# ZeayW/Multimodal-fusion-based-Pre-routing-Timing-Prediction-

Measured on AMD Instinct MI355X. Metric: train-step samples/sec, higher is better.
Workload: dtype bf16; 1 GPU; config B: 8 designs/step/GPU, 65536-node netlist, 64 levels, 256x256 tile, 1350 endpoints/design, UNet(max), bf16 operands / fp32 accumulate on the MFMA-bound contractions; U-Net activations and their gradients stored bf16, netlist tensors, statistics, parameters and gradients fp32; nodes=65536, levels=64, tile=256, endpoints_per_design=1350, cone_pruning=False, parallelism=dp1 (designs sharded, one all-reduce of the flat gradient per step), launch=one HIP graph replay per step (Adam inside)

## Files before the change

multimodal-fusion-based-pre-routing-timing-prediction-_amd/csrc/mlp_feat.hip:

```cpp
#include <stdlib.h>
#include "mlp_tile_bf16.h"
#include "tr_read.h"

namespace mmft {

int launch_slab_reduce(const float* slabs, int splits, long long elems, float* out, int accumulate, hipStream_t st);

__device__ __forceinline__ unsigned short mf_bf16(float v) { return (unsigned short)(pack_bf16(v, 0.f) & 0xffff); }

__device__ __forceinline__ bf16x8 mf_pack8(const float* v) {
  u32x4 p = {pack_bf16(v[0], v[1]), pack_bf16(v[2], v[3]), pack_bf16(v[4], v[5]), pack_bf16(v[6], v[7])};
  return __builtin_bit_cast(bf16x8, p);
}

__device__ __forceinline__ bf16x8 mf_w1_frag(const float* __restrict__ w1, int fin, int col, int k0) {
  float v[8];
#pragma unroll
  for (int t = 0; t < 8; ++t) v[t] = k0 + t < fin ? w1[(long long)col * fin + k0 + t] : 0.f;
  return mf_pack8(v);
}

struct FeatFwdArgs {
  const float* x;
  long long ldx;
  int row0, n, fin;
  const float *w1, *b1, *w2, *b2;
  float* out;
  long long ldout;
  int relu_out;
};

template <int KS>
__global__ void __launch_bounds__(512) mlp2_feat_fwd_kernel(FeatFwdArgs a) {
  constexpr int BM = 64, RT = BM / 16, XS = KS * 32 + 8, HS = L2_HD + 8;
  __shared__ __attribute__((aligned(16))) unsigned short xs[BM * XS];
  __shared__ __attribute__((aligned(16))) unsigned short hs[BM * HS];
  const int tid = threadIdx.x, lane = tid & 63, wave = tid >> 6;
  const int r16 = lane & 15, q = lane >> 4;
  bf16x8 w1f[2][KS], w2f[8];
#pragma unroll
  for (int j = 0; j < 2; ++j)
#pragma unroll
    for (int ks = 0; ks < KS; ++ks) w1f[j][ks] = mf_w1_frag(a.w1, a.fin, wave * 32 + j * 16 + r16, ks * 32 + q * 8);
#pragma unroll
  for (int ks = 0; ks < 8; ++ks) w2f[ks] = mf_pack8(a.w2 + (long long)(wave * 16 + r16) * L2_HD + ks * 32 + q * 8);
  const int nn2 = wave * 16 + q * 4;
  const f32x4 b2v = *reinterpret_cast<const f32x4*>(a.b2 + nn2);
  f32x4 b1v[2];
#pragma unroll
  for (int j = 0; j < 2; ++j) b1v[j] = *reinterpret_cast<const f32x4*>(a.b1 + wave * 32 + j * 16 + q * 4);
  constexpr int NXE = BM * KS * 32 / 512;
  float xr[NXE];
  auto request = [&](int tile) {
#pragma unroll
    for (int k = 0; k < NXE; ++k) {
      const int e = tid + k * 512, r = e / (KS * 32), kk = e % (KS * 32);
      const int m = tile * BM + r;
      xr[k] = (m < a.n && kk < a.fin) ? a.x[(long long)(a.row0 + m) * a.ldx + kk] : 0.f;
    }
  };
  const int ntiles = (a.n + BM - 1) / BM;
  if ((int)blockIdx.x < ntiles) request(blockIdx.x);
  for (int tile = blockIdx.x; tile < ntiles; tile += gridDim.x) {
    const int m0 = tile * BM;
#pragma unroll
    for (int k = 0; k < NXE; ++k) {
      const int e = tid + k * 512;
      xs[(e / (KS * 32)) * XS + e % (KS * 32)] = mf_bf16(xr[k]);
    }
    __syncthreads();
    if (tile + (int)gridDim.x < ntiles) request(tile + gridDim.x);
    f32x4 acc1[RT][2];
    tile_layer1<KS, RT>(acc1, w1f, xs, XS, r16, q);
#pragma unroll
    for (int i = 0; i < RT; ++i)
#pragma unroll
      for (int j = 0; j < 2; ++j) st_bf16x4(hs + (i * 16 + r16) * HS + wave * 32 + j * 16 + q * 4, relu4(acc1[i][j] + b1v[j]));
    __syncthreads();
    f32x4 acc2[RT];
#pragma unroll
    for (int i = 0; i < RT; ++i) acc2[i] = tile_layer2(w2f, hs, HS, r16, q, i);
#pragma unroll
    for (int i = 0; i < RT; ++i) {
      const int m = m0 + i * 16 + r16;
      if (m >= a.n) continue;
      f32x4 v = acc2[i] + b2v;
      if (a.relu_out) v = relu4(v);
      *reinterpret_cast<f32x4*>(a.out + (long long)(a.row0 + m) * a.ldout + nn2) = v;
    }
    __syncthreads();
  }
}

struct FeatBwdArgs {
  const float* g;
  long long ldg;
  const float* x;
  long long ldx;
  int row0, n, fin;
  const float *w1, *b1, *w2;
  float* slabs;
  long long slab;
};

template <int KS>
__global__ void __launch_bounds__(512) mlp2_feat_bwd_kernel(FeatBwdArgs a) {
  constexpr int BM = 32, KP = KS * 32, XS = KP + 16, GS = L2_D2 + 16, HS = L2_HD + 16, KB = KP / 16;
  extern __shared__ __attribute__((aligned(16))) unsigned short lds[];
  unsigned short* xs = lds;
  unsigned short* gs = xs + BM * XS;
  unsigned short* hs = gs + BM * GS;
  unsigned short* ds = hs + BM * HS;
  f32x4(*gred)[32] = reinterpret_cast<f32x4(*)[32]>(hs);
  const int tid = threadIdx.x, lane = tid & 63, wave = tid >> 6;
  const int r16 = lane & 15, q = lane >> 4;
  const int trr = tr_lane_row(lane), trc = tr_lane_col(lane);
  const f32x4 zero = {0.f, 0.f, 0.f, 0.f};

  bf16x8 w1f[2][KS], w2tf[2][4];
  f32x4 b1v[2];
#pragma unroll
  for (int j = 0; j < 2; ++j) {
    const int col = wave * 32 + j * 16 + r16;
#pragma unroll
    for (int ks = 0; ks < KS; ++ks) w1f[j][ks] = mf_w1_frag(a.w1, a.fin, col, ks * 32 + q * 8);
#pragma unroll
    for (int ks = 0; ks < 4; ++ks) {
      float v[8];
#pragma unroll
      for (int t = 0; t < 8; ++t) v[t] = a.w2[(long long)(ks * 32 + q * 8 + t) * L2_HD + col];
      w2tf[j][ks] = mf_pack8(v);
    }
    b1v[j] = *reinterpret_cast<const f32x4*>(a.b1 + wave * 32 + j * 16 + q * 4);
  }
  f32x4 dw2[2][8], dw1[2][KB], dsum[2], gsum = zero;
#pragma unroll
  for (int j = 0; j < 2; ++j) {
    dsum[j] = zero;
#pragma unroll
    for (int d = 0; d < 8; ++d) dw2[j][d] = zero;
#pragma unroll
    for (int k = 0; k < KB; ++k) dw1[j][k] = zero;
  }

  const int ntiles = (a.n + BM - 1) / BM;
  constexpr int NXE = BM * KP / 512;
  f32x4 gr[2];
  float xr[NXE];
  auto request = [&](int tile) {
    const int m0 = tile * BM;
#pragma unroll
    for (int it = 0; it < 2; ++it) {
      const int e = tid + it * 512, r = e >> 5, c = (e & 31) * 4;
      gr[it] = m0 + r < a.n ? *reinterpret_cast<const f32x4*>(a.g + (long long)(a.row0 + m0 + r) * a.ldg + c) : zero;
    }
#pragma unroll
    for (int k = 0; k < NXE; ++k) {
      const int e = tid + k * 512, r = e / KP, kk = e % KP;
      xr[k] = (m0 + r < a.n && kk < a.fin) ? a.x[(long long)(a.row0 + m0 + r) * a.ldx + kk] : 0.f;
    }
  };
  if ((int)blockIdx.x < ntiles) request(blockIdx.x);
  for (int tile = blockIdx.x; tile < ntiles; tile += gridDim.x) {
#pragma unroll
    for (int it = 0; it < 2; ++it) {
      const int e = tid + it * 512, r = e >> 5, c = (e & 31) * 4;
      const f32x4 v = gr[it];
      gsum += v;
      const unsigned lo = pack_bf16(v.x, v.y), hi = pack_bf16(v.z, v.w);
      *reinterpret_cast<unsigned long long*>(gs + r * GS + c) = ((unsigned long long)hi << 32) | lo;
    }
#pragma unroll
    for (int k = 0; k < NXE; ++k) {
      const int e = tid + k * 512, r = e / KP, kk = e % KP;
      xs[r * XS + kk] = mf_bf16(xr[k]);
    }
    __syncthreads();
    if (tile + (int)gridDim.x < ntiles) request(tile + gridDim.x);
    __syncthreads();
#pragma unroll
    for (int i = 0; i < 2; ++i) {
      f32x4 acc1[2] = {zero, zero}, acc3[2] = {zero, zero};
#pragma unroll
      for (int ks = 0; ks < KS; ++ks) {
        const bf16x8 xf = *reinterpret_cast<const bf16x8*>(xs + (i * 16 + r16) * XS + ks * 32 + q * 8);
#pragma unroll
        for (int j = 0; j < 2; ++j) acc1[j] = __builtin_amdgcn_mfma_f32_16x16x32_bf16(w1f[j][ks], xf, acc1[j], 0, 0, 0);
      }
#pragma unroll
      for (int ks = 0; ks < 4; ++ks) {
        const bf16x8 gf = *reinterpret_cast<const bf16x8*>(gs + (i * 16 + r16) * GS + ks * 32 + q * 8);
#pragma unroll
        for (int j = 0; j < 2; ++j) acc3[j] = __builtin_amdgcn_mfma_f32_16x16x32_bf16(w2tf[j][ks], gf, acc3[j], 0, 0, 0);
      }
      const int m = i * 16 + r16;
#pragma unroll
      for (int j = 0; j < 2; ++j) {
        const int nn = wave * 32 + j * 16 + q * 4;
        f32x4 hv = acc1[j] + b1v[j], dh = acc3[j];
#pragma unroll
        for (int t = 0; t < 4; ++t) {
          hv[t] = hv[t] > 0.f ? hv[t] : 0.f;
          dh[t] = hv[t] > 0.f ? dh[t] : 0.f;
        }
        dsum[j] += dh;
        const unsigned hl = pack_bf16(hv.x, hv.y), hh = pack_bf16(hv.z, hv.w);
        const unsigned dl = pack_bf16(dh.x, dh.y), dhh = pack_bf16(dh.z, dh.w);
        *reinterpret_cast<unsigned long long*>(hs + m * HS + nn) = ((unsigned long long)hh << 32) | hl;
        *reinterpret_cast<unsigned long long*>(ds + m * HS + nn) = ((unsigned long long)dhh << 32) | dl;
      }
    }
    __syncthreads();
#pragma unroll
    for (int j = 0; j < 2; ++j) {
      const int col0 = wave * 32 + j * 16;
      const bf16x8 hf = __builtin_bit_cast(bf16x8, tr_read_pair(hs + trr * HS + col0 + trc, 16 * HS));
      const bf16x8 df = __builtin_bit_cast(bf16x8, tr_read_pair(ds + trr * HS + col0 + trc, 16 * HS));
#pragma unroll
      for (int d = 0; d < 8; ++d) {
        const bf16x8 gf = __builtin_bit_cast(bf16x8, tr_read_pair(gs + trr * GS + d * 16 + trc, 16 * GS));
        dw2[j][d] = __builtin_amdgcn_mfma_f32_16x16x32_bf16(hf, gf, dw2[j][d], 0, 0, 0);
      }
#pragma unroll
      for (int k = 0; k < KB; ++k) {
        const bf16x8 xf = __builtin_bit_cast(bf16x8, tr_read_pair(xs + trr * XS + k * 16 + trc, 16 * XS));
        dw1[j][k] = __builtin_amdgcn_mfma_f32_16x16x32_bf16(df, xf, dw1[j][k], 0, 0, 0);
      }
    }
    __syncthreads();
  }

  float* sl = a.slabs + (long long)blockIdx.x * a.slab;
  float* s_dw1 = sl;
  float* s_db1 = s_dw1 + (long long)L2_HD * a.fin;
  float* s_dw2 = s_db1 + L2_HD;
  float* s_db2 = s_dw2 + (long long)L2_D2 * L2_HD;
#pragma unroll
  for (int j = 0; j < 2; ++j) {
    const int colq = wave * 32 + j * 16 + q * 4;
#pragma unroll
    for (int d = 0; d < 8; ++d) *reinterpret_cast<f32x4*>(s_dw2 + (long long)(d * 16 + r16) * L2_HD + colq) = dw2[j][d];
#pragma unroll
    for (int k = 0; k < KB; ++k) {
      const int kk = k * 16 + r16;
      if (kk < a.fin) {
#pragma unroll
        for (int t = 0; t < 4; ++t) s_dw1[(long long)(colq + t) * a.fin + kk] = dw1[j][k][t];
      }
    }
    f32x4 v = dsum[j];
#pragma unroll
    for (int o = 1; o < 16; o <<= 1) {
#pragma unroll
      for (int t = 0; t < 4; ++t) v[t] += __shfl_xor(v[t], o, 64);
    }
    if (r16 == 0) *reinterpret_cast<f32x4*>(s_db1 + colq) = v;
  }
  __syncthreads();
  gred[tid >> 5][tid & 31] = gsum;
  __syncthreads();
  if (tid < 32) {
    f32x4 v = gred[0][tid];
    for (int p = 1; p < 16; ++p) v += gred[p][tid];
    *reinterpret_cast<f32x4*>(s_db2 + tid * 4) = v;
  }
}

template <int KS>
constexpr int feat_bwd_lds() {
  constexpr int BM = 32, KP = KS * 32, XS = KP + 16, GS = L2_D2 + 16, HS = L2_HD + 16;
  return (BM * XS + BM * GS + 2 * BM * HS) * 2;
}

static inline long long feat_slab(int fin) { return (long long)L2_HD * fin + L2_HD + (long long)L2_D2 * L2_HD + L2_D2; }
static inline int feat_bwd_grid(int n) {
  int tiles = cdiv(n, 32);
  static int cap = getenv("MMFT_FEAT_BWD_GRID") ? atoi(getenv("MMFT_FEAT_BWD_GRID")) : 192;
  if (cap < 1) cap = 1;
  return tiles < cap ? (tiles < 1 ? 1 : tiles) : cap;
}

}

using namespace mmft;

extern "C" int mmft_mlp2_feat_fwd_bf16(const float* x, long long ldx, int row0, int n, int fin, const float* w1, const float* b1,
                                       const float* w2, const float* b2, float* out, long long ldout, int relu_out, int device,
                                       void* stream) {
  MMFT_REQUIRE(x && w1 && b1 && w2 && b2 && out, "mlp2_feat_fwd_bf16: null pointer");
  MMFT_REQUIRE(n >= 0 && row0 >= 0 && fin >= 1 && fin <= 64 && ldx >= fin, "mlp2_feat_fwd_bf16: bad sizes (fin <= 64)");
  MMFT_REQUIRE(ldout % 4 == 0 && aligned16(out) && aligned16(w2) && aligned16(b1) && aligned16(b2),
               "mlp2_feat_fwd_bf16: out / w2 / biases must be 16-byte aligned");
  if (n == 0) return MMFT_OK;
  DeviceGuard dg(device);
  FeatFwdArgs a{x, ldx, row0, n, fin, w1, b1, w2, b2, out, ldout, relu_out};
  const double fl = 2.0 * n * ((double)fin * L2_HD + (double)L2_HD * L2_D2), by = 4.0 * n * ((double)fin + L2_D2);
  int grid = cdiv(n, 64);
  if (grid > 768) grid = 768;
  if (fin <= 32)
    MMFT_LAUNCH("mlp2_feat_fwd_kernel", fl, by, mlp2_feat_fwd_kernel<1>, dim3(grid), dim3(512), (hipStream_t)stream, a);
  else
    MMFT_LAUNCH("mlp2_feat_fwd_kernel", fl, by, mlp2_feat_fwd_kernel<2>, dim3(grid), dim3(512), (hipStream_t)stream, a);
  return check_launch("mlp2_feat_fwd_bf16");
}

extern "C" long long mmft_mlp2_feat_bwd_workspace_bytes(int n, int fin) {
  if (n <= 0 || fin < 1 || fin > 64) return 0;
  return (long long)feat_bwd_grid(n) * feat_slab(fin) * 4;
}

extern "C" int mmft_mlp2_feat_bwd_bf16(const float* g, long long ldg, const float* x, long long ldx, int row0, int n, int fin,
                                       const float* w1, const float* b1, const float* w2, float* dw1, float* db1, float* dw2,
                                       float* db2, int accumulate, float* workspace, long long workspace_bytes, int device,
                                       void* stream) {
  MMFT_REQUIRE(g && x && w1 && b1 && w2 && dw1 && db1 && dw2 && db2, "mlp2_feat_bwd_bf16: null pointer");
  MMFT_REQUIRE(n > 0 && row0 >= 0 && fin >= 1 && fin <= 64 && ldx >= fin && ldg >= L2_D2, "mlp2_feat_bwd_bf16: bad sizes (fin <= 64)");
  MMFT_REQUIRE(ldg % 4 == 0 && aligned16(g) && aligned16(b1), "mlp2_feat_bwd_bf16: g / b1 must be 16-byte aligned");
  MMFT_REQUIRE(workspace && aligned16(workspace) && workspace_bytes >= mmft_mlp2_feat_bwd_workspace_bytes(n, fin),
               "mlp2_feat_bwd_bf16: workspace too small");
  DeviceGuard dg(device);
  hipStream_t st = (hipStream_t)stream;
  const int grid = feat_bwd_grid(n);
  const long long slab = feat_slab(fin);
  FeatBwdArgs a{g, ldg, x, ldx, row0, n, fin, w1, b1, w2, workspace, slab};
  const double fl = 2.0 * n * (2.0 * fin * L2_HD + 2.0 * L2_HD * L2_D2), by = 4.0 * n * ((double)fin + L2_D2);
  static DynLdsOnce once[2];
  int arc = fin <= 32 ? ensure_dyn_lds(once[0], reinterpret_cast<const void*>(&mlp2_feat_bwd_kernel<1>), feat_bwd_lds<1>(), "mlp2_feat_bwd_bf16")
                      : ensure_dyn_lds(once[1], reinterpret_cast<const void*>(&mlp2_feat_bwd_kernel<2>), feat_bwd_lds<2>(), "mlp2_feat_bwd_bf16");
  if (arc) return arc;
  if (fin <= 32)
    MMFT_LAUNCH_LDS("mlp2_feat_bwd_kernel", fl, by, mlp2_feat_bwd_kernel<1>, dim3(grid), dim3(512), feat_bwd_lds<1>(), st, a);
  else
    MMFT_LAUNCH_LDS("mlp2_feat_bwd_kernel", fl, by, mlp2_feat_bwd_kernel<2>, dim3(grid), dim3(512), feat_bwd_lds<2>(), st, a);
  int rc = check_launch("mlp2_feat_bwd_bf16");
  if (rc) return rc;
  if (db1 == dw1 + (long long)L2_HD * fin && dw2 == db1 + L2_HD && db2 == dw2 + (long long)L2_D2 * L2_HD && aligned16(dw1))
    return launch_slab_reduce(workspace, grid, slab, dw1, accumulate, st);
  const long long o1 = (long long)L2_HD * fin, o2 = o1 + L2_HD, o3 = o2 + (long long)L2_D2 * L2_HD;
  const SlabSeg segs[4] = {{workspace, dw1, slab, grid, (int)o1, 1, accumulate ? 1 : 0},
                           {workspace + o1, db1, slab, grid, L2_HD, 1, accumulate ? 1 : 0},
                           {workspace + o2, dw2, slab, grid, L2_D2 * L2_HD, 1, accumulate ? 1 : 0},
                           {workspace + o3, db2, slab, grid, L2_D2, 1, accumulate ? 1 : 0}};
  return launch_slab_reduce_batch(segs, 4, st);
}
```

Measured before the change: 2403 designs/s.

## Double-buffer feature-MLP input tiles with vectorized loads and trimmed K blocks

Stages the feature-MLP input tiles through double-buffered LDS using a new XStage helper. When x is contiguous and aligned it loads with 16-byte vector reads, and it deposits the next tile while the current tile's layer-2 or weight-gradient work runs, which removes one barrier per tile. The backward kernel is now templated on the number of live 16-wide K blocks so dw1 accumulators scale with fin, and for KS=2 it moves the W2^T fragments into LDS to cut register pressure. The forward grid cap and launch bounds also change. The cost is more LDS per block, extra bookkeeping, and added complexity in boundary handling.

```diff
diff --git a/multimodal-fusion-based-pre-routing-timing-prediction-_amd/csrc/mlp_feat.hip b/multimodal-fusion-based-pre-routing-timing-prediction-_amd/csrc/mlp_feat.hip
--- a/multimodal-fusion-based-pre-routing-timing-prediction-_amd/csrc/mlp_feat.hip
+++ b/multimodal-fusion-based-pre-routing-timing-prediction-_amd/csrc/mlp_feat.hip
@@ -18,6 +18,77 @@
 #pragma unroll
   for (int t = 0; t < 8; ++t) v[t] = k0 + t < fin ? w1[(long long)col * fin + k0 + t] : 0.f;
   return mf_pack8(v);
+}
+
+template <int BM, int XS, int KL>
+struct XStage {
+  static constexpr int XTILE = BM * XS + 8;
+  static constexpr int NV = (BM * KL / 4 + 511) / 512, NS = BM * KL / 512, NR = 4 * NV > NS ? 4 * NV : NS;
+  float r[NR];
+  unsigned off[NV][2];
+
+  __device__ __forceinline__ void init(int tid, int fin) {
+#pragma unroll
+    for (int k = 0; k < NV; ++k)
+#pragma unroll
+      for (int h = 0; h < 2; ++h) {
+        unsigned w = 0;
+#pragma unroll
+        for (int t = 0; t < 2; ++t) {
+          const int e = 4 * (tid + k * 512) + 2 * h + t;
+          const unsigned o = e < BM * fin ? (unsigned)((e / fin) * XS + e % fin) : (unsigned)(BM * XS);
+          w |= o << (16 * t);
+        }
+        off[k][h] = w;
+      }
+  }
+  static __device__ __forceinline__ int live(int m0, int n, int fin) { return (n - m0 < BM ? n - m0 : BM) * fin; }
+  __device__ __forceinline__ void request(const float* __restrict__ x, long long ldx, int row0, int m0, int n, int fin, int vec, int tid) {
+    if (vec) {
+      const int lim = live(m0, n, fin);
+      const float* xb = x + (long long)(row0 + m0) * fin;
+#pragma unroll
+      for (int k = 0; k < NV; ++k) {
+        const int e0 = 4 * (tid + k * 512);
+        const bool full = e0 + 4 <= lim;
+        const f32x4 v = *reinterpret_cast<const f32x4*>(full ? xb + e0 : x + (long long)row0 * fin);
+        r[4 * k] = v.x; r[4 * k + 1] = v.y; r[4 * k + 2] = v.z; r[4 * k + 3] = v.w;
+        if (!full && e0 < lim) {
+#pragma unroll
+          for (int t = 0; t < 4; ++t) r[4 * k + t] = e0 + t < lim ? xb[e0 + t] : 0.f;
+        }
+      }
+    } else {
+#pragma unroll
+      for (int k = 0; k < NS; ++k) {
+        const int e = tid + k * 512, rr = e / KL, kk = e % KL;
+        r[k] = (m0 + rr < n && kk < fin) ? x[(long long)(row0 + m0 + rr) * ldx + kk] : 0.f;
+      }
+    }
+  }
+  __device__ __forceinline__ void deposit(unsigned short* xs, int m0, int n, int fin, int vec, int tid) const {
+    if (vec) {
+      const int lim = live(m0, n, fin);
+#pragma unroll
+      for (int k = 0; k < NV; ++k) {
+        if (4 * (tid + k * 512) >= BM * fin) continue;
+#pragma unroll
+        for (int t = 0; t < 4; ++t) {
+          const int e = 4 * (tid + k * 512) + t;
+          xs[(off[k][t >> 1] >> (16 * (t & 1))) & 0xffffu] = mf_bf16(e < lim ? r[4 * k + t] : 0.f);
+        }
+      }
+    } else {
+#pragma unroll
+      for (int k = 0; k < NS; ++k) {
+        const int e = tid + k * 512, rr = e / KL, kk = e % KL;
+        if (kk < fin) xs[rr * XS + kk] = mf_bf16(r[k]);
+      }
+    }
+  }
+};
+static inline int feat_x_vec(const float* x, long long ldx, int row0, int n, int fin) {
+  return ldx == fin && ((long long)row0 * fin) % 4 == 0 && (long long)n * fin >= 4 && (reinterpret_cast<uintptr_t>(x) & 15) == 0;
 }
 
 struct FeatFwdArgs {
@@ -27,16 +98,23 @@
   const float *w1, *b1, *w2, *b2;
   float* out;
   long long ldout;
-  int relu_out;
+  int relu_out, xvec;
 };
 
 template <int KS>
-__global__ void __launch_bounds__(512) mlp2_feat_fwd_kernel(FeatFwdArgs a) {
+__global__ void __launch_bounds__(512, KS == 1 ? 4 : 2) mlp2_feat_fwd_kernel(FeatFwdArgs a) {
   constexpr int BM = 64, RT = BM / 16, XS = KS * 32 + 8, HS = L2_HD + 8;
-  __shared__ __attribute__((aligned(16))) unsigned short xs[BM * XS];
+  using XQ = XStage<BM, XS, KS * 32>;
+  __shared__ __attribute__((aligned(16))) unsigned short xs[2][XQ::XTILE];
   __shared__ __attribute__((aligned(16))) unsigned short hs[BM * HS];
   const int tid = threadIdx.x, lane = tid & 63, wave = tid >> 6;
   const int r16 = lane & 15, q = lane >> 4;
+  const int ntiles = (a.n + BM - 1) / BM, G = gridDim.x;
+  if ((int)blockIdx.x >= ntiles) return;
+  XQ xq;
+  xq.init(tid, a.fin);
+  xq.request(a.x, a.ldx, a.row0, blockIdx.x * BM, a.n, a.fin, a.xvec, tid);
+  for (int e = tid; e < 2 * XQ::XTILE / 2; e += 512) reinterpret_cast<unsigned*>(&xs[0][0])[e] = 0u;
   bf16x8 w1f[2][KS], w2f[8];
 #pragma unroll
   for (int j = 0; j < 2; ++j)
@@ -49,42 +127,34 @@
   f32x4 b1v[2];
 #pragma unroll
   for (int j = 0; j < 2; ++j) b1v[j] = *reinterpret_cast<const f32x4*>(a.b1 + wave * 32 + j * 16 + q * 4);
-  constexpr int NXE = BM * KS * 32 / 512;
-  float xr[NXE];
-  auto request = [&](int tile) {
-#pragma unroll
-    for (int k = 0; k < NXE; ++k) {
-      const int e = tid + k * 512, r = e / (KS * 32), kk = e % (KS * 32);
-      const int m = tile * BM + r;
-      xr[k] = (m < a.n && kk < a.fin) ? a.x[(long long)(a.row0 + m) * a.ldx + kk] : 0.f;
-    }
-  };
-  const int ntiles = (a.n + BM - 1) / BM;
-  if ((int)blockIdx.x < ntiles) request(blockIdx.x);
-  for (int tile = blockIdx.x; tile < ntiles; tile += gridDim.x) {
+  __syncthreads();
+  xq.deposit(xs[0], blockIdx.x * BM, a.n, a.fin, a.xvec, tid);
+  if ((int)blockIdx.x + G < ntiles) xq.request(a.x, a.ldx, a.row0, (blockIdx.x + G) * BM, a.n, a.fin, a.xvec, tid);
+  __syncthreads();
+  int buf = 0;
+  for (int tile = blockIdx.x; tile < ntiles; tile += G, buf ^= 1) {
     const int m0 = tile * BM;
 #pragma unroll
-    for (int k = 0; k < NXE; ++k) {
-      const int e = tid + k * 512;
-      xs[(e / (KS * 32)) * XS + e % (KS * 32)] = mf_bf16(xr[k]);
+    for (int h = 0; h < RT / 2; ++h) {
+      f32x4 acc1[2][2];
+      tile_layer1<KS, 2>(acc1, w1f, xs[buf] + h * 32 * XS, XS, r16, q);
+#pragma unroll
+      for (int i = 0; i < 2; ++i)
+#pragma unroll
+        for (int j = 0; j < 2; ++j)
+          st_bf16x4(hs + (h * 32 + i * 16 + r16) * HS + wave * 32 + j * 16 + q * 4, relu4(acc1[i][j] + b1v[j]));
     }
     __syncthreads();
-    if (tile + (int)gridDim.x < ntiles) request(tile + gridDim.x);
-    f32x4 acc1[RT][2];
-    tile_layer1<KS, RT>(acc1, w1f, xs, XS, r16, q);
-#pragma unroll
-    for (int i = 0; i < RT; ++i)
-#pragma unroll
-      for (int j = 0; j < 2; ++j) st_bf16x4(hs + (i * 16 + r16) * HS + wave * 32 + j * 16 + q * 4, relu4(acc1[i][j] + b1v[j]));
-    __syncthreads();
-    f32x4 acc2[RT];
-#pragma unroll
-    for (int i = 0; i < RT; ++i) acc2[i] = tile_layer2(w2f, hs, HS, r16, q, i);
+    if (tile + G < ntiles) {
+      xq.deposit(xs[buf ^ 1], (tile + G) * BM, a.n, a.fin, a.xvec, tid);
+      if (tile + 2 * G < ntiles) xq.request(a.x, a.ldx, a.row0, (tile + 2 * G) * BM, a.n, a.fin, a.xvec, tid);
+    }
 #pragma unroll
     for (int i = 0; i < RT; ++i) {
+      const f32x4 acc2 = tile_layer2(w2f, hs, HS, r16, q, i);
       const int m = m0 + i * 16 + r16;
       if (m >= a.n) continue;
-      f32x4 v = acc2[i] + b2v;
+      f32x4 v = acc2 + b2v;
       if (a.relu_out) v = relu4(v);
       *reinterpret_cast<f32x4*>(a.out + (long long)(a.row0 + m) * a.ldout + nn2) = v;
     }
@@ -101,23 +171,28 @@
   const float *w1, *b1, *w2;
   float* slabs;
   long long slab;
+  int xvec;
 };
 
-template <int KS>
+template <int KS, int KB>
 __global__ void __launch_bounds__(512) mlp2_feat_bwd_kernel(FeatBwdArgs a) {
-  constexpr int BM = 32, KP = KS * 32, XS = KP + 16, GS = L2_D2 + 16, HS = L2_HD + 16, KB = KP / 16;
+  constexpr int BM = 32, KP = KS * 32, XS = KP + 16, GS = L2_D2 + 16, HS = L2_HD + 16;
+  static_assert(KB == 2 * KS - 1 || KB == 2 * KS, "KB: live 16-blocks of the KS K steps");
   extern __shared__ __attribute__((aligned(16))) unsigned short lds[];
-  unsigned short* xs = lds;
-  unsigned short* gs = xs + BM * XS;
-  unsigned short* hs = gs + BM * GS;
+  unsigned short* xs0 = lds;
+  using XQ = XStage<BM, XS, KB * 16>;
+  unsigned short* gs0 = xs0 + 2 * XQ::XTILE;
+  unsigned short* hs = gs0 + 2 * BM * GS;
   unsigned short* ds = hs + BM * HS;
+  constexpr bool W2L = KS == 2;
+  bf16x8* w2l = reinterpret_cast<bf16x8*>(ds + BM * HS) + (threadIdx.x >> 6) * 8 * 64 + (threadIdx.x & 63);
   f32x4(*gred)[32] = reinterpret_cast<f32x4(*)[32]>(hs);
   const int tid = threadIdx.x, lane = tid & 63, wave = tid >> 6;
   const int r16 = lane & 15, q = lane >> 4;
   const int trr = tr_lane_row(lane), trc = tr_lane_col(lane);
   const f32x4 zero = {0.f, 0.f, 0.f, 0.f};
 
-  bf16x8 w1f[2][KS], w2tf[2][4];
+  bf16x8 w1f[2][KS], w2tf[W2L ? 1 : 2][W2L ? 1 : 4];
   f32x4 b1v[2];
 #pragma unroll
   for (int j = 0; j < 2; ++j) {
@@ -129,7 +204,8 @@
       float v[8];
 #pragma unroll
       for (int t = 0; t < 8; ++t) v[t] = a.w2[(long long)(ks * 32 + q * 8 + t) * L2_HD + col];
-      w2tf[j][ks] = mf_pack8(v);
+      if constexpr (W2L) w2l[(j * 4 + ks) * 64] = mf_pack8(v);
+      else w2tf[j][ks] = mf_pack8(v);
     }
     b1v[j] = *reinterpret_cast<const f32x4*>(a.b1 + wave * 32 + j * 16 + q * 4);
   }
@@ -143,10 +219,10 @@
     for (int k = 0; k < KB; ++k) dw1[j][k] = zero;
   }
 
-  const int ntiles = (a.n + BM - 1) / BM;
-  constexpr int NXE = BM * KP / 512;
+  const int ntiles = (a.n + BM - 1) / BM, G = gridDim.x;
   f32x4 gr[2];
-  float xr[NXE];
+  XQ xq;
+  xq.init(tid, a.fin);
   auto request = [&](int tile) {
     const int m0 = tile * BM;
 #pragma unroll
@@ -154,14 +230,10 @@
       const int e = tid + it * 512, r = e >> 5, c = (e & 31) * 4;
       gr[it] = m0 + r < a.n ? *reinterpret_cast<const f32x4*>(a.g + (long long)(a.row0 + m0 + r) * a.ldg + c) : zero;
     }
-#pragma unroll
-    for (int k = 0; k < NXE; ++k) {
-      const int e = tid + k * 512, r = e / KP, kk = e % KP;
-      xr[k] = (m0 + r < a.n && kk < a.fin) ? a.x[(long long)(a.row0 + m0 + r) * a.ldx + kk] : 0.f;
-    }
+    xq.request(a.x, a.ldx, a.row0, m0, a.n, a.fin, a.xvec, tid);
   };
-  if ((int)blockIdx.x < ntiles) request(blockIdx.x);
-  for (int tile = blockIdx.x; tile < ntiles; tile += gridDim.x) {
+  auto deposit = [&](int tile, int b) {
+    unsigned short* gs = gs0 + b * BM * GS;
 #pragma unroll
     for (int it = 0; it < 2; ++it) {
       const int e = tid + it * 512, r = e >> 5, c = (e & 31) * 4;
@@ -170,34 +242,70 @@
       const unsigned lo = pack_bf16(v.x, v.y), hi = pack_bf16(v.z, v.w);
       *reinterpret_cast<unsigned long long*>(gs + r * GS + c) = ((unsigned long long)hi << 32) | lo;
     }
-#pragma unroll
-    for (int k = 0; k < NXE; ++k) {
-      const int e = tid + k * 512, r = e / KP, kk = e % KP;
-      xs[r * XS + kk] = mf_bf16(xr[k]);
-    }
-    __syncthreads();
-    if (tile + (int)gridDim.x < ntiles) request(tile + gridDim.x);
-    __syncthreads();
+    xq.deposit(xs0 + b * XQ::XTILE, tile * BM, a.n, a.fin, a.xvec, tid);
+  };
+  if ((int)blockIdx.x < ntiles) request(blockIdx.x);
+  for (int e = tid; e < 2 * XQ::XTILE / 2; e += 512) reinterpret_cast<unsigned*>(xs0)[e] = 0u;
+  __syncthreads();
+  if ((int)blockIdx.x < ntiles) {
+    deposit(blockIdx.x, 0);
+    if ((int)blockIdx.x + G < ntiles) request(blockIdx.x + G);
+  }
+  __syncthreads();
+  int buf = 0;
+  for (int tile = blockIdx.x; tile < ntiles; tile += G, buf ^= 1) {
+    const unsigned short* xs = xs0 + buf * XQ::XTILE;
+    const unsigned short* gs = gs0 + buf * BM * GS;
+    f32x4 acc1[2][2], acc3[2][2];
+#pragma unroll
+    for (int i = 0; i < 2; ++i)
+#pragma unroll
+      for (int j = 0; j < 2; ++j) acc1[i][j] = acc3[i][j] = zero;
+    if constexpr (W2L) {
+#pragma unroll
+      for (int ks = 0; ks < KS; ++ks)
+#pragma unroll
+        for (int i = 0; i < 2; ++i) {
+          const bf16x8 xf = *reinterpret_cast<const bf16x8*>(xs + (i * 16 + r16) * XS + ks * 32 + q * 8);
+#pragma unroll
+          for (int j = 0; j < 2; ++j) acc1[i][j] = __builtin_amdgcn_mfma_f32_16x16x32_bf16(w1f[j][ks], xf, acc1[i][j], 0, 0, 0);
+        }
+#pragma unroll
+      for (int ks = 0; ks < 4; ++ks) {
+        bf16x8 wf[2];
+#pragma unroll
+        for (int j = 0; j < 2; ++j) wf[j] = w2l[(j * 4 + ks) * 64];
+#pragma unroll
+        for (int i = 0; i < 2; ++i) {
+          const bf16x8 gf = *reinterpret_cast<const bf16x8*>(gs + (i * 16 + r16) * GS + ks * 32 + q * 8);
+#pragma unroll
+          for (int j = 0; j < 2; ++j) acc3[i][j] = __builtin_amdgcn_mfma_f32_16x16x32_bf16(wf[j], gf, acc3[i][j], 0, 0, 0);
+        }
+      }
+    } else {
+#pragma unroll
+      for (int i = 0; i < 2; ++i) {
+#pragma unroll
+        for (int ks = 0; ks < KS; ++ks) {
+          const bf16x8 xf = *reinterpret_cast<const bf16x8*>(xs + (i * 16 + r16) * XS + ks * 32 + q * 8);
+#pragma unroll
+          for (int j = 0; j < 2; ++j) acc1[i][j] = __builtin_amdgcn_mfma_f32_16x16x32_bf16(w1f[j][ks], xf, acc1[i][j], 0, 0, 0);
+        }
+#pragma unroll
+        for (int ks = 0; ks < 4; ++ks) {
+          const bf16x8 gf = *reinterpret_cast<const bf16x8*>(gs + (i * 16 + r16) * GS + ks * 32 + q * 8);
+#pragma unroll
+          for (int j = 0; j < 2; ++j) acc3[i][j] = __builtin_amdgcn_mfma_f32_16x16x32_bf16(w2tf[j][ks], gf, acc3[i][j], 0, 0, 0);
+        }
+      }
+    }
 #pragma unroll
     for (int i = 0; i < 2; ++i) {
-      f32x4 acc1[2] = {zero, zero}, acc3[2] = {zero, zero};
-#pragma unroll
-      for (int ks = 0; ks < KS; ++ks) {
-        const bf16x8 xf = *reinterpret_cast<const bf16x8*>(xs + (i * 16 + r16) * XS + ks * 32 + q * 8);
-#pragma unroll
-        for (int j = 0; j < 2; ++j) acc1[j] = __builtin_amdgcn_mfma_f32_16x16x32_bf16(w1f[j][ks], xf, acc1[j], 0, 0, 0);
-      }
-#pragma unroll
-      for (int ks = 0; ks < 4; ++ks) {
-        const bf16x8 gf = *reinterpret_cast<const bf16x8*>(gs + (i * 16 + r16) * GS + ks * 32 + q * 8);
-#pragma unroll
-        for (int j = 0; j < 2; ++j) acc3[j] = __builtin_amdgcn_mfma_f32_16x16x32_bf16(w2tf[j][ks], gf, acc3[j], 0, 0, 0);
-      }
       const int m = i * 16 + r16;
 #pragma unroll
       for (int j = 0; j < 2; ++j) {
         const int nn = wave * 32 + j * 16 + q * 4;
-        f32x4 hv = acc1[j] + b1v[j], dh = acc3[j];
+        f32x4 hv = acc1[i][j] + b1v[j], dh = acc3[i][j];
 #pragma unroll
         for (int t = 0; t < 4; ++t) {
           hv[t] = hv[t] > 0.f ? hv[t] : 0.f;
@@ -211,6 +319,10 @@
       }
     }
     __syncthreads();
+    if (tile + G < ntiles) {
+      deposit(tile + G, buf ^ 1);
+      if (tile + 2 * G < ntiles) request(tile + 2 * G);
+    }
 #pragma unroll
     for (int j = 0; j < 2; ++j) {
       const int col0 = wave * 32 + j * 16;
@@ -269,7 +381,7 @@
 template <int KS>
 constexpr int feat_bwd_lds() {
   constexpr int BM = 32, KP = KS * 32, XS = KP + 16, GS = L2_D2 + 16, HS = L2_HD + 16;
-  return (BM * XS + BM * GS + 2 * BM * HS) * 2;
+  return (2 * (BM * XS + 8) + 2 * BM * GS + 2 * BM * HS) * 2 + (KS == 2 ? L2_HD * L2_D2 * 2 : 0);
 }
 
 static inline long long feat_slab(int fin) { return (long long)L2_HD * fin + L2_HD + (long long)L2_D2 * L2_HD + L2_D2; }
@@ -278,6 +390,15 @@
   static int cap = getenv("MMFT_FEAT_BWD_GRID") ? atoi(getenv("MMFT_FEAT_BWD_GRID")) : 192;
   if (cap < 1) cap = 1;
   return tiles < cap ? (tiles < 1 ? 1 : tiles) : cap;
+}
+
+template <int KS, int KB>
+static int feat_bwd_launch(const FeatBwdArgs& a, int grid, double fl, double by, hipStream_t st) {
+  static DynLdsOnce once;
+  const auto kernel = &mlp2_feat_bwd_kernel<KS, KB>;
+  if (int rc = ensure_dyn_lds(once, reinterpret_cast<const void*>(kernel), feat_bwd_lds<KS>(), "mlp2_feat_bwd_bf16")) return rc;
+  MMFT_LAUNCH_LDS("mlp2_feat_bwd_kernel", fl, by, kernel, dim3(grid), dim3(512), feat_bwd_lds<KS>(), st, a);
+  return check_launch("mlp2_feat_bwd_bf16");
 }
 
 }
@@ -293,10 +414,11 @@
                "mlp2_feat_fwd_bf16: out / w2 / biases must be 16-byte aligned");
   if (n == 0) return MMFT_OK;
   DeviceGuard dg(device);
-  FeatFwdArgs a{x, ldx, row0, n, fin, w1, b1, w2, b2, out, ldout, relu_out};
+  FeatFwdArgs a{x, ldx, row0, n, fin, w1, b1, w2, b2, out, ldout, relu_out, feat_x_vec(x, ldx, row0, n, fin)};
   const double fl = 2.0 * n * ((double)fin * L2_HD + (double)L2_HD * L2_D2), by = 4.0 * n * ((double)fin + L2_D2);
+  const int cap = fin <= 32 ? 512 : 256;
   int grid = cdiv(n, 64);
-  if (grid > 768) grid = 768;
+  if (grid > cap) grid = cap;
   if (fin <= 32)
     MMFT_LAUNCH("mlp2_feat_fwd_kernel", fl, by, mlp2_feat_fwd_kernel<1>, dim3(grid), dim3(512), (hipStream_t)stream, a);
   else
@@ -322,17 +444,11 @@
   hipStream_t st = (hipStream_t)stream;
   const int grid = feat_bwd_grid(n);
   const long long slab = feat_slab(fin);
-  FeatBwdArgs a{g, ldg, x, ldx, row0, n, fin, w1, b1, w2, workspace, slab};
+  FeatBwdArgs a{g, ldg, x, ldx, row0, n, fin, w1, b1, w2, workspace, slab, feat_x_vec(x, ldx, row0, n, fin)};
   const double fl = 2.0 * n * (2.0 * fin * L2_HD + 2.0 * L2_HD * L2_D2), by = 4.0 * n * ((double)fin + L2_D2);
-  static DynLdsOnce once[2];
-  int arc = fin <= 32 ? ensure_dyn_lds(once[0], reinterpret_cast<const void*>(&mlp2_feat_bwd_kernel<1>), feat_bwd_lds<1>(), "mlp2_feat_bwd_bf16")
-                      : ensure_dyn_lds(once[1], reinterpret_cast<const void*>(&mlp2_feat_bwd_kernel<2>), feat_bwd_lds<2>(), "mlp2_feat_bwd_bf16");
-  if (arc) return arc;
-  if (fin <= 32)
-    MMFT_LAUNCH_LDS("mlp2_feat_bwd_kernel", fl, by, mlp2_feat_bwd_kernel<1>, dim3(grid), dim3(512), feat_bwd_lds<1>(), st, a);
-  else
-    MMFT_LAUNCH_LDS("mlp2_feat_bwd_kernel", fl, by, mlp2_feat_bwd_kernel<2>, dim3(grid), dim3(512), feat_bwd_lds<2>(), st, a);
-  int rc = check_launch("mlp2_feat_bwd_bf16");
+  const int kb = cdiv(fin, 16);
+  int rc = kb == 1 ? feat_bwd_launch<1, 1>(a, grid, fl, by, st) : kb == 2 ? feat_bwd_launch<1, 2>(a, grid, fl, by, st)
+         : kb == 3 ? feat_bwd_launch<2, 3>(a, grid, fl, by, st) : feat_bwd_launch<2, 4>(a, grid, fl, by, st);
   if (rc) return rc;
   if (db1 == dw1 + (long long)L2_HD * fin && dw2 == db1 + L2_HD && db2 == dw2 + (long long)L2_D2 * L2_HD && aligned16(dw1))
     return launch_slab_reduce(workspace, grid, slab, dw1, accumulate, st);
```

After: 2408 designs/s (median of 4 runs). Within noise of the previous version (+0.2%).
